# SavaRobotics/FoundationPose

Hardware: AMD Instinct MI355X
Metric: pose-hypotheses/sec (render+refine+score), 252 hyp x 160x160 (higher is better)
Workload: dtype f16

## Files before the change

foundationpose_amd/_lib.py:

```python
import ctypes
import os
import weakref
from ctypes import POINTER, Structure, byref, c_char_p, c_double, c_float, c_int, c_int64, c_uint, c_void_p

import numpy as np
import torch

_HERE = os.path.dirname(os.path.abspath(__file__))
LIB_PATH = os.path.join(_HERE, 'lib', 'libfoundationpose_amd.so')
_lib = None

FP_REFINE_SHARED_TRANSLATION = 1
FP_NET_REFINE, FP_NET_SCORE = 0, 1
FP_EINVAL = -1
FP_ERR_ADD, FP_ERR_ADDS, FP_ERR_ADD_SYM = 1, 2, 4
FP_BOP_MSSD, FP_BOP_MSPD = 1, 2
FP_VSD_MAX_TAUS = 32
FP_MESH_DIAMETER_MAX_POINTS = 1 << 21
FP_MESH_SIMPLIFY_MAX_VERTICES, FP_MESH_SIMPLIFY_MAX_FACES = 1 << 21, 1 << 23
FP_MESH_COMPONENTS_MAX_VERTICES, FP_MESH_COMPONENTS_MAX_FACES = 1 << 21, 1 << 23
FP_SCENE_MAX_INSTANCES = 1024
FP_SCENE_OCC_DEPTH, FP_SCENE_OCC_INSTANCES = 1, 2
FP_SCENE_INFO_COLS = 12
FP_SCENE_INFO_PX_COUNT_ALL, FP_SCENE_INFO_PX_COUNT_VALID, FP_SCENE_INFO_PX_COUNT_VISIB, FP_SCENE_INFO_PX_COUNT_IN_FRAME = 0, 1, 2, 3
# ... 138 lines not shown
  'fp_tsdf_integrate': (c_int, [c_void_p, c_void_p, c_void_p, c_void_p, c_void_p, c_int, c_int, c_int, c_void_p, c_void_p, c_float, c_void_p]),
  'fp_tsdf_extract_count': (c_int, [c_void_p, c_void_p, c_float, c_void_p, c_void_p]),
  'fp_tsdf_extract_write': (c_int, [c_void_p, c_void_p, c_void_p, c_void_p, c_void_p, c_void_p, c_int64, c_int64, c_void_p]),
  'fp_tsdf_read_plane': (c_int, [c_void_p, c_void_p, c_int, c_void_p, c_void_p]),
  'fp_tsdf_align': (c_int, [c_void_p, c_void_p, c_void_p, c_void_p, c_int, c_int, c_int, c_void_p, c_void_p, c_float, c_float, c_void_p, c_void_p, c_void_p]),
  'fp_texture_bake': (c_int, [c_void_p, c_void_p, c_int, c_void_p, c_int, c_void_p, c_void_p, c_void_p, c_void_p, c_int, c_int, c_int, c_void_p, c_void_p,
                              POINTER(FpTextureCfg), c_void_p, c_void_p, c_void_p, c_void_p]),
  'fp_point_mesh_distance': (c_int, [c_void_p, c_void_p, c_int, c_void_p, c_int, c_void_p, c_int, c_void_p, c_void_p, c_void_p, c_void_p]),
  'fp_distance_stats': (c_int, [c_void_p, c_void_p, c_int, c_void_p, c_int, c_void_p, c_void_p]),
  'fp_mesh_sample_surface': (c_int, [c_void_p, c_void_p, c_int, c_void_p, c_int, c_int, c_uint, c_void_p, c_void_p, c_void_p, c_void_p, c_void_p]),
  'fp_net_create': (c_int, [c_void_p, c_int, POINTER(FpTensor), c_int, c_int, POINTER(c_void_p)]),
  'fp_net_destroy': (c_int, [c_void_p]),
  'fp_net_rot_dim': (c_int, [c_void_p]),
  'fp_refine_forward': (c_int, [c_void_p, c_void_p, c_void_p, c_int, c_void_p, c_void_p, c_void_p]),
  'fp_net_tokens': (c_int, [c_void_p, c_void_p, c_void_p, c_int, c_void_p, c_void_p]),
  'fp_score_features': (c_int, [c_void_p, c_void_p, c_void_p, c_int, c_void_p, c_void_p]),
  'fp_score_tail': (c_int, [c_void_p, c_void_p, c_void_p, c_int, c_int, c_void_p, c_void_p, c_void_p]),
  'fp_score_tail_scores': (c_int, [c_void_p, c_void_p, c_void_p, c_int, c_int, c_int, c_float, c_void_p, c_void_p, c_void_p, c_void_p]),
  'fp_score_predict_rows_multi': (c_int, [c_void_p, c_void_p, POINTER(FpObjectBatch), c_int, c_double, c_int, c_void_p, c_void_p, c_void_p]),
  'fp_track_frame': (c_int, [c_void_p, POINTER(FpTrackArgs), c_void_p]),
  'fp_track_objects': (c_int, [c_void_p, POINTER(FpTrackObjectsArgs), c_void_p]),
  'fp_register_objects': (c_int, [c_void_p, POINTER(FpRegisterObjectsArgs), c_void_p]),
  'fp_mask_depth_stats_objects': (c_int, [c_void_p, c_void_p, c_void_p, c_void_p, c_void_p, c_int, c_int, c_int, c_float, c_void_p, c_void_p, c_void_p]),
  'fp_register_hypotheses': (c_int, [c_void_p, c_void_p, c_void_p, c_int, c_void_p, c_void_p, c_void_p, c_void_p, c_void_p]),
  'fp_register_rank': (c_int, [c_void_p, c_void_p, c_void_p, c_void_p, c_int, c_void_p, c_void_p, c_void_p, c_void_p, c_void_p, c_void_p]),
  'fp_pose_update': (c_int, [c_void_p, c_void_p, c_void_p, c_void_p, c_int, c_int, c_int, c_void_p, c_float, c_float, c_void_p, c_void_p]),
  'fp_pose_update_deepim': (c_int, [c_void_p, c_void_p, c_void_p, c_void_p, c_int, c_int, c_void_p, c_void_p, c_float, c_float, c_float, c_void_p, c_void_p]),
  'fp_refine_predict': (c_int, [c_void_p, c_void_p, c_void_p, c_void_p, c_void_p, c_int, c_int, c_void_p, c_double, POINTER(FpRefineCfg), c_void_p, c_int, c_int, c_void_p, c_void_p, c_void_p]),
  'fp_refine_predict_multi': (c_int, [c_void_p, c_void_p, POINTER(FpObjectBatch), c_int, POINTER(FpRefineCfg), c_void_p, c_int, c_void_p, c_void_p, c_void_p]),
  'fp_refine_predict_multi_flags': (c_int, [c_void_p, c_void_p, POINTER(FpObjectBatch), c_int, POINTER(FpRefineCfg), c_void_p, c_int, c_void_p, c_void_p, c_uint, c_void_p]),
  'fp_score_predict_features_multi': (c_int, [c_void_p, c_void_p, POINTER(FpObjectBatch), c_int, c_double, c_int, c_void_p, c_void_p, c_void_p]),
  'fp_score_predict_features': (c_int, [c_void_p, c_void_p, c_void_p, c_void_p, c_void_p, c_int, c_int, c_void_p, c_double, c_double, c_int, c_void_p, c_int, c_void_p, c_void_p]),
  'fp_conv3x3_band_f16': (c_int, [c_void_p, c_void_p, c_int, c_int, c_void_p, c_void_p, c_void_p, c_int, c_void_p, c_void_p]),
  'fp_conv2d_f16': (c_int, [c_void_p, c_void_p, c_int, c_int, c_int, c_int, c_void_p, c_void_p, c_int, c_int, c_int, c_int, c_int, c_void_p, c_int, c_void_p, c_int, c_void_p]),
  'fp_token_linear_f16': (c_int, [c_void_p, c_void_p, c_int, c_void_p, c_void_p, c_int, c_int, c_void_p, c_void_p, c_void_p, c_int, c_void_p, c_void_p]),
  'fp_head_mlp_f16': (c_int, [c_void_p, c_void_p, c_void_p, c_int] + [c_void_p] * 8 + [c_void_p, c_void_p]),
  'fp_attention_f16': (c_int, [c_void_p, c_void_p, c_void_p, c_int, c_int, c_void_p, c_void_p]),
  'fp_cluster_poses': (c_int, [c_float, c_float, c_void_p, c_int, c_void_p, c_int, c_void_p]),
  'fp_prof_enable': (c_int, [c_void_p, c_int]),
  'fp_prof_read': (c_int, [c_void_p, c_char_p, POINTER(c_double), POINTER(c_int64), POINTER(c_double)]),
  'fp_prof_read_busy': (c_int, [c_void_p, c_char_p, POINTER(c_double)]),
  'fp_prof_reset': (c_int, [c_void_p]),
}


def exported_symbols():
  return sorted(_PROTOS)


def lib():
  global _lib
  if _lib is None:
    if not os.path.exists(LIB_PATH):
      raise FoundationPoseAmdError(
        f'{LIB_PATH} is missing: build the HIP library first (python -c "import __graft_entry__ as g; g.build()" '
        f'or make -C foundationpose_amd/csrc).  foundationpose_amd has no CPU fallback.')
    L = ctypes.CDLL(LIB_PATH)
    for name, (res, args) in _PROTOS.items():
      fn = getattr(L, name)
      fn.restype = res
      fn.argtypes = args
    _lib = L
  return _lib


def check(rc):
# ... 180 lines not shown
```

foundationpose_amd/csrc/api.hip:

```cpp
#include "common.h"
#include <memory>
#include <cstring>

#include <cmath>
#include <cstdarg>
#include <cstdlib>
#include <algorithm>

static thread_local char g_err[1024] = "";

void fp_set_error(const char *fmt, ...) {
  va_list ap;
  va_start(ap, fmt);
  vsnprintf(g_err, sizeof(g_err), fmt, ap);
  va_end(ap);
}

extern "C" const char *fp_last_error(void) { return g_err; }
extern "C" int fp_version(void) { return 102; }

size_t fp_arena_bytes_for(int n_hyp) {
  return (size_t)n_hyp * (size_t)(17u << 20) + ((size_t)64 << 20);
}

size_t fp_arena_inner_bytes(int n_hyp) {
  return (size_t)n_hyp * (size_t)(15u << 20) + ((size_t)8 << 20) + (n_hyp <= 4 ? ((size_t)40 << 20) : 0);
}

int fp_arena_ensure(fp_ctx *ctx, size_t bytes) {
  Arena &a = ctx->arena;
  if (a.cap - a.off >= bytes && a.base) return FP_OK;
  if (a.off != 0) {
    fp_set_error("arena too small for a nested request of %zu bytes (cap %zu, used %zu); call fp_ctx_reserve first", bytes, a.cap, a.off);
    return FP_ENOMEM;
  }
  FP_CHECK_HIP(hipSetDevice(ctx->device));
  if (a.base) {
    FP_CHECK_HIP(hipDeviceSynchronize());
    FP_CHECK_HIP(hipFree(a.base));
    a.base = nullptr;
    a.cap = 0;
  }
  void *p = nullptr;
  hipError_t e = hipMalloc(&p, bytes);
  if (e != hipSuccess) {
    fp_set_error("hipMalloc(%zu) failed: %s", bytes, hipGetErrorString(e));
    return FP_ENOMEM;
  }
  a.base = (char *)p;
  a.cap = bytes;
  a.off = 0;
  ++a.generation;
  return FP_OK;
}

int fp_set_kernel_attributes(fp_ctx *ctx) {
  std::vector<KernelLds> v;
  conv_kernel_lds(v), conv_halo_kernel_lds(v), conv_s1b_kernel_lds(v), conv_small_kernel_lds(v), conv_s2_kernel_lds(v), stem_kernel_lds(v);
  tok_gemm_kernel_lds(v), tok_qkv_kernel_lds(v), head_mlp_kernel_lds(v), attn_kernel_lds(v), raster_kernel_lds(v);
  FP_CHECK_HIP(hipSetDevice(ctx->device));
  for (const KernelLds &k : v)
    if (k.bytes > 48 * 1024) FP_CHECK_HIP(hipFuncSetAttribute(k.fn, hipFuncAttributeMaxDynamicSharedMemorySize, k.bytes));
  return FP_OK;
}

extern "C" int fp_ctx_create(int device, fp_ctx **out) {
  FP_REQUIRE(out, "fp_ctx_create: null out");
  int n = 0;
  FP_CHECK_HIP(hipGetDeviceCount(&n));
  FP_REQUIRE(device >= 0 && device < n, "fp_ctx_create: device %d out of range (%d visible)", device, n);
  FP_CHECK_HIP(hipSetDevice(device));
  hipDeviceProp_t prop;
  FP_CHECK_HIP(hipGetDeviceProperties(&prop, device));
  fp_ctx *c = new fp_ctx;
  c->device = device;
  c->num_cu = prop.multiProcessorCount;
  if (hipMalloc(&c->zero_page, 4096 + FP_TAIL_MAX_GROUPS * sizeof(int)) != hipSuccess ||
      hipMemset(c->zero_page, 0, 4096 + FP_TAIL_MAX_GROUPS * sizeof(int)) != hipSuccess) {
    delete c;
    fp_set_error("fp_ctx_create: zero page allocation failed");
    return FP_ENOMEM;
  }
  c->tail_counter = (int *)((char *)c->zero_page + 4096);
  const int rc = fp_set_kernel_attributes(c);
  if (rc != FP_OK) {
    (void)hipFree(c->zero_page);
    delete c;
    return rc;
  }
  *out = c;
  return FP_OK;
// ... 1223 lines not shown
                             int Cout, int KH, int KW, int stride, int pad, const void *d_res, int relu, void *d_out, int out_f32,
                             void *stream) {
  FP_REQUIRE(ctx && d_in && d_w_packed && d_bias && d_out, "fp_conv2d_f16: null argument");
  FP_REQUIRE(stride >= 1 && pad >= 0 && Nimg >= 0, "fp_conv2d_f16: bad stride/pad/N");
  ConvArgs a = conv_args(d_in, d_w_packed, d_bias, d_res, d_out, Nimg, H, W, Cin, Cout, KH, KW, stride, pad, relu);
  a.out_mode = out_f32 ? 1 : 0;
  ArenaScope scope(ctx->arena);
  if (!out_f32 && conv_small_shape(a, ctx->num_cu)) {
    const size_t bytes = small_packed_halfs(Cout, Cin) * sizeof(f16);
    FP_TRY(fp_arena_ensure(ctx, bytes + 4096));
    f16 *pk = (f16 *)ctx->arena.take(bytes);
    if (!pk) return FP_ENOMEM;
    FP_TRY(small_pack_weights(a.w, Cout, Cin, a.Kpad, pk, (hipStream_t)stream));
    a.wsm = pk;
    return launch_conv(ctx, a, (hipStream_t)stream);
  }
  a.ksplit = out_f32 ? 0 : conv_ksplit(a, ctx->num_cu);
  if (a.ksplit > 1) {
    const size_t bytes = (size_t)a.ksplit * a.M * a.Cout * sizeof(float);
    FP_TRY(fp_arena_ensure(ctx, bytes + 4096));
    a.splitk = (float *)ctx->arena.take(bytes);
    return a.splitk ? launch_conv(ctx, a, (hipStream_t)stream) : FP_ENOMEM;
  }
  a.ksplit = 0;
  if (!out_f32 && a.M >= S2_MIN_PIXELS && s2_supported(a)) {
    const size_t bytes = s2_packed_halfs(Cout, Cin) * sizeof(f16);
    FP_TRY(fp_arena_ensure(ctx, bytes + 4096));
    f16 *pk = (f16 *)ctx->arena.take(bytes);
    if (!pk) return FP_ENOMEM;
    FP_TRY(s2_pack_weights(a.w, Cout, Cin, a.Kpad, pk, (hipStream_t)stream));
    a.wpk = pk;
    return launch_conv(ctx, a, (hipStream_t)stream);
  }
  return launch_conv(ctx, a, (hipStream_t)stream);
}

extern "C" int fp_conv3x3_band_f16(fp_ctx *ctx, const void *d_in, int Nimg, int C, const void *d_w_packed, const float *d_bias, const void *d_res,
                                   int relu, void *d_out, void *stream) {
  FP_REQUIRE(ctx && d_in && d_w_packed && d_bias && d_out && Nimg >= 0, "fp_conv3x3_band_f16: bad argument");
  FP_REQUIRE(C == 128 || C == 256, "fp_conv3x3_band_f16: C=%d (128 or 256)", C);
  ConvArgs a = conv_args(d_in, d_w_packed, d_bias, d_res, d_out, Nimg, 40, 40, C, C, 3, 3, 1, 1, relu);
  if (a.M == 0) return FP_OK;
  const size_t bytes = s2_packed_halfs(C, C) * sizeof(f16);
  FP_TRY(fp_arena_ensure(ctx, bytes + 4096));
  ArenaScope scope(ctx->arena);
  f16 *pk = (f16 *)ctx->arena.take(bytes);
  if (!pk) return FP_ENOMEM;
  FP_TRY(s2_pack_weights(a.w, C, C, a.Kpad, pk, (hipStream_t)stream, 2, 1));
  a.wpk = pk;
  return launch_conv_s1b(ctx, a, (hipStream_t)stream);
}

extern "C" int fp_attention_f16(fp_ctx *ctx, const void *d_qk, const void *d_vt, int B, int T, void *d_out, void *stream) {
  FP_REQUIRE(ctx && d_qk && d_vt && d_out, "fp_attention_f16: null argument");
  return launch_attention(ctx, (const f16 *)d_qk, (const f16 *)d_vt, B, T, (f16 *)d_out, (hipStream_t)stream);
}

extern "C" int fp_cluster_poses(float angle_diff_deg, float dist_diff_m, const float *in, int n_in, const float *sym, int n_sym,
                                float *out) {
  FP_REQUIRE(in && sym && out && n_in >= 1 && n_sym >= 1, "fp_cluster_poses: bad argument");
  const float radian_thres = angle_diff_deg / 180.0f * (float)M_PI;
  int n_out = 0;
  auto keep = [&](const float *p) {
    memcpy(out + (size_t)n_out * 16, p, 16 * sizeof(float));
    ++n_out;
  };
  keep(in);
// ... 28 lines not shown
```

foundationpose_amd/csrc/common.h:

```cpp
#pragma once
#include <hip/hip_runtime.h>
#include <stdint.h>
#include <stdio.h>
#include <stdlib.h>
#include <string.h>
#include <string>
#include <vector>
#include <map>

#include "../../include/foundationpose_amd.h"

typedef _Float16 f16;
typedef _Float16 half8 __attribute__((ext_vector_type(8)));
typedef _Float16 half4 __attribute__((ext_vector_type(4)));
typedef float floatx16 __attribute__((ext_vector_type(16)));
typedef float floatx4 __attribute__((ext_vector_type(4)));

void fp_set_error(const char *fmt, ...);

inline long long fp_env_int(const char *name, long long fallback) {
  const char *e = getenv(name);
  return e ? atoll(e) : fallback;
}
inline bool fp_env_set(const char *name) { return getenv(name) != nullptr; }
// ... 173 lines not shown
    if (!ctx->ev_pool.empty()) {
      e = ctx->ev_pool.back();
      ctx->ev_pool.pop_back();
    } else {
      (void)hipEventCreate(&e);
    }
    return e;
  }
  ~ProfScope() {
    if (on) {
      (void)hipEventRecord(ev.b, s);
      ctx->pending.push_back(ev);
    }
  }
};

#ifdef __HIPCC__
__device__ __forceinline__ int xcd_remap(int id, int nwg) {
  const int xcd = id & 7, slot = id >> 3;
  const int q = nwg >> 3, r = nwg & 7;
  return (xcd < r ? xcd * (q + 1) : r * (q + 1) + (xcd - r) * q) + slot;
}
#endif

struct KernelLds {
  const void *fn;
  int bytes;
};
void conv_kernel_lds(std::vector<KernelLds> &v);
void conv_halo_kernel_lds(std::vector<KernelLds> &v);
void conv_s1b_kernel_lds(std::vector<KernelLds> &v);
void conv_small_kernel_lds(std::vector<KernelLds> &v);
void conv_s2_kernel_lds(std::vector<KernelLds> &v);
void stem_kernel_lds(std::vector<KernelLds> &v);
void tok_gemm_kernel_lds(std::vector<KernelLds> &v);
void tok_qkv_kernel_lds(std::vector<KernelLds> &v);
void head_mlp_kernel_lds(std::vector<KernelLds> &v);
void attn_kernel_lds(std::vector<KernelLds> &v);
void raster_kernel_lds(std::vector<KernelLds> &v);
int fp_set_kernel_attributes(fp_ctx *ctx);

struct ConvArgs {
  const f16 *in;
  const f16 *w;
  const float *bias;
  const f16 *res;
  const float *post_add;
  void *out;
  int Nimg, H, W, Cin, Ho, Wo, Cout, KH, KW, stride, pad, Kpad, M;
  int relu, out_mode;
  int out_ld, split_m, coff_hi, post_period, tokens;
  float *splitk = nullptr;
  int ksplit = 0;
  const f16 *wpk = nullptr;
  const f16 *wsm = nullptr;
  int hyp = 0;
};
int launch_conv(fp_ctx *ctx, const ConvArgs &a, hipStream_t s);
#define S2_MIN_PIXELS 2000
bool s2_supported(const ConvArgs &a);
int s2_ct_for(int Cout);
size_t s2_packed_halfs(int Cout, int Cin);
int s2_pack_weights(const f16 *d_w, int Cout, int Cin, int Kpad, f16 *d_out, hipStream_t s, int ct_force = 0, int order = 0);
int launch_conv_s2(fp_ctx *ctx, const ConvArgs &a, hipStream_t s);
bool s1b_supported(const ConvArgs &a);
int launch_conv_s1b(fp_ctx *ctx, const ConvArgs &a, hipStream_t s);

bool conv_small_shape(const ConvArgs &a, int num_cu);
bool conv_small_use(const ConvArgs &a, int num_cu);
size_t small_packed_halfs(int Cout, int Cin);
int small_pack_weights(const f16 *d_w, int Cout, int Cin, int Kpad, f16 *d_out, hipStream_t s);
int launch_conv_small(fp_ctx *ctx, const ConvArgs &a, hipStream_t s);

__host__ __device__ __forceinline__ int vt_col(int t) { return (t & ~15) | (((t >> 2) & 1) << 3) | (((t >> 3) & 1) << 2) | (t & 3); }
int launch_attention(fp_ctx *ctx, const f16 *qk, const f16 *vt, int B, int T, f16 *out, hipStream_t s);

#define TG_MAXBLK 6
struct TokGemmBlock {
  const f16 *w;
  const float *bias;
  void *out;
  int ld, coff;
  int relu;
  int vt = 0;
};
struct TokGemmArgs {
  const f16 *in;
  int M, nblk, tokens;
  TokGemmBlock blk[TG_MAXBLK];
  const f16 *res;
  const float *gamma, *beta;
  float *gsum;
};
enum { TG_EPI_ROWS = 0, TG_EPI_VT = 1, TG_EPI_LN = 2, TG_EPI_LNSUM = 3 };
int launch_tok_gemm(fp_ctx *ctx, const TokGemmArgs &a, int epi, hipStream_t s);
int tok_qkv_small_max();
int launch_tok_qkv(fp_ctx *ctx, const TokGemmArgs &a, hipStream_t s, int hyp = 0);
// ... 166 lines not shown
```

foundationpose_amd/csrc/conv.hip:

```cpp
#include "common.h"
#include "device_util.h"
#include <cstdlib>
#include <type_traits>

#define CV_BK 32

#define C2_BN 256
#define C2_BK 32

#ifdef HALO_STAMP
__device__ unsigned long long g_igemm_stamps[4096 * 4 * 4];
extern "C" __attribute__((visibility("default"))) int fp_dbg_igemm_stamps(unsigned long long *host) {
  return hipMemcpyFromSymbol(host, HIP_SYMBOL(g_igemm_stamps), sizeof(g_igemm_stamps)) == hipSuccess ? 0 : -1;
}
#define ISTAMP(x) x
#else
#define ISTAMP(x)
#endif


template <int BM, int KW, bool CIN8, int NT, bool RES, bool SPLIT = false>
__device__ __forceinline__ void igemm2_tile(const ConvArgs &p, const f16 *__restrict__ zero_page, const int m0, const int c0, f16 *smem, const int ks = 0) {
  constexpr int TN = 64 * NT;
  constexpr int XH = TN * C2_BK, WH = BM * C2_BK;
// ... 410 lines not shown

bool conv_halo_supported(const ConvArgs &a);
int launch_conv_halo(fp_ctx *ctx, const ConvArgs &a, hipStream_t s);
bool stem_supported(const ConvArgs &a);
int launch_stem(fp_ctx *ctx, const ConvArgs &a, hipStream_t s);

int launch_conv(fp_ctx *ctx, const ConvArgs &a, hipStream_t s) {
  FP_REQUIRE(a.Cin == 8 || a.Cin % 32 == 0, "conv: Cin=%d must be 8 or a multiple of 32", a.Cin);
  FP_REQUIRE(a.Cout % 64 == 0, "conv: Cout=%d must be a multiple of 64", a.Cout);
  FP_REQUIRE(a.Kpad % CV_BK == 0 && a.Kpad >= a.KH * a.KW * a.Cin, "conv: bad Kpad=%d", a.Kpad);
  FP_REQUIRE(a.KH == a.KW && (a.KW == 1 || a.KW == 3 || a.KW == 7), "conv: kernel %dx%d unsupported (1,3,7)", a.KH, a.KW);
  FP_REQUIRE(a.M == a.Nimg * a.Ho * a.Wo, "conv: M mismatch");
  FP_REQUIRE(a.out_ld % 4 == 0 && a.coff_hi % 4 == 0, "conv: out_ld/coff must be multiples of 4");
  if (a.M == 0) return FP_OK;
  const double flops = 2.0 * (double)a.M * a.Cout * a.KH * a.KW * (a.Cin == 8 ? 6 : a.Cin);
  const bool halo = conv_halo_supported(a);
  const char *cls = halo ? "conv3x3_halo" : (a.KW == 3) ? "conv3x3_s2" : (a.KW == 7 ? "conv7x7" : "linear");
  ProfScope ps(ctx, s, cls, flops);
  if (!(a.splitk && a.ksplit > 1) && conv_small_use(a, ctx->num_cu)) return launch_conv_small(ctx, a, s);
  {
    static const int band = fp_env_int("FP_C128_BAND", 1);
    if (band != 0 && (a.Cin == 128 || band == 2) && (long long)a.M > (long long)ctx->num_cu * 512 && s1b_supported(a)) return launch_conv_s1b(ctx, a, s);
  }
  if (halo) return launch_conv_halo(ctx, a, s);
  if (a.splitk && a.ksplit > 1) {
    FP_REQUIRE(a.KW == 3 && a.stride == 2 && a.Cout % 128 == 0 && (a.Kpad / C2_BK) % a.ksplit == 0 && a.out_mode == 0, "conv split-K: unsupported layer");
    const int n_t = ((a.M + 63) / 64) * (a.Cout / 128);
    hipLaunchKernelGGL((conv_igemm2_splitk_kernel<128, 3>), dim3(n_t * a.ksplit), dim3(256), igemm2_lds_bytes<128>(), s, a, (const f16 *)ctx->zero_page);
    FP_CHECK_HIP(hipGetLastError());
    return launch_splitk_finish(a, s);
  }
  if (stem_supported(a)) return launch_stem(ctx, a, s);
  if (a.wpk && a.M >= S2_MIN_PIXELS && s2_supported(a)) return launch_conv_s2(ctx, a, s);
  const bool bm128 = (a.Cout % 128 == 0);
  const f16 *zp = (const f16 *)ctx->zero_page;
  if (a.Cin == 8) {
    FP_REQUIRE(a.KW == 7, "conv: Cin=8 path is the 7x7 stem");
    return bm128 ? launch_two<128, 7, true>(ctx, a, zp, s) : launch_two<64, 7, true>(ctx, a, zp, s);
  }
  if (a.KW == 3) return bm128 ? launch_two<128, 3, false>(ctx, a, zp, s) : launch_two<64, 3, false>(ctx, a, zp, s);
  if (a.KW == 1) return bm128 ? launch_two<128, 1, false>(ctx, a, zp, s) : launch_two<64, 1, false>(ctx, a, zp, s);
  FP_REQUIRE(false, "conv: unsupported configuration KW=%d Cin=%d", a.KW, a.Cin);
}
```

foundationpose_amd/csrc/conv_s2.hip:

```cpp
#include "common.h"
#include "device_util.h"

#define S2_THREADS 256
#define S2_STAGE_PAD 8

template <int WO, int ROWS, int CT>
struct S2Cfg {
  static constexpr int P = 42;
  static_assert(WO == 20, "pitch chosen for 20-wide outputs");
  static constexpr int BROWS = 2 * ROWS + 2;
  static constexpr int NPT = ROWS * WO / 32;
  static constexpr int BAND_INSTR = ((BROWS * P + 31) / 32 + 3) / 4 * 4;
  static constexpr int BAND_BYTES = BAND_INSTR * 1024;
  static constexpr int DPW = BAND_INSTR / 4;
  static constexpr int STAGE_LD = CT * 32 + S2_STAGE_PAD;
  static constexpr int LDS_BYTES = 2 * BAND_BYTES;
  static_assert(ROWS * WO == NPT * 32 && (2 * P - WO) % 16 == 0 && P >= 2 * WO + 1, "tile / pitch");
  static_assert(4 * 32 * STAGE_LD * 2 <= BAND_BYTES, "epilogue staging fits one band buffer");
};

__global__ void s2_pack_kernel(const f16 *__restrict__ w, int Cin, int Kpad, int CT, size_t total, f16 *__restrict__ out, int order) {
  const size_t idx = (size_t)blockIdx.x * blockDim.x + threadIdx.x;
  if (idx >= total) return;
  const int e = idx & 7, lane = (idx >> 3) & 63;
  size_t rest = idx >> 9;
  const int nch = Cin / 16;
  const int ct = rest % CT;
  rest /= CT;
  int tap, chunk;
  if (order == 1) {
    const int ks = rest % 2;
    rest /= 2;
    tap = rest % 9;
    rest /= 9;
    chunk = (int)(rest % (nch / 2)) * 2 + ks;
    rest /= nch / 2;
  } else {
    tap = rest % 9;
    rest /= 9;
    chunk = rest % nch;
    rest /= nch;
  }
  const int co = ((int)rest * CT + ct) * 32 + (lane & 31);
  const int k = tap * Cin + chunk * 16 + (lane >> 5) * 8 + e;
  out[idx] = w[(size_t)co * Kpad + k];
}

template <int WO, int ROWS, int CT>
__global__ __launch_bounds__(S2_THREADS, 2) void conv3x3_s2_kernel(ConvArgs p, const f16 *__restrict__ wpk, const f16 *__restrict__ zero_page,
                                                                    int n_tiles, int n_cob) {
  using C = S2Cfg<WO, ROWS, CT>;
  constexpr int HO = WO, HI = 2 * WO, WI = 2 * WO, P = C::P, NPT = C::NPT, DPW = C::DPW;
  extern __shared__ __attribute__((aligned(16))) unsigned char s2_smem[];
  const int tid = threadIdx.x, lane = tid & 63, wave = __builtin_amdgcn_readfirstlane(tid >> 6);
  const int lr = lane & 31, lh = lane >> 5;
  const unsigned lds0 = (unsigned)(size_t)(__attribute__((address_space(3))) void *)s2_smem;

  const int tile = xcd_remap(blockIdx.x, n_tiles);
  const int cb = tile % n_cob, pt = tile / n_cob;
  const int g0 = pt * ROWS;
  const int img0 = g0 / HO, oy0 = g0 - img0 * HO;
  const int jb = HO - oy0;
  const int nch = p.Cin >> 4;

  unsigned src_off[DPW];
#pragma unroll
  for (int v = 0; v < DPW; ++v) {
    const int q = (wave + 4 * v) * 32 + (lane >> 1), hl = (lane & 1) ^ ((q >> 3) & 1);
    const int b = q / P, c = q - b * P;
// ... 156 lines not shown
```

foundationpose_amd/csrc/net.hip:

```cpp
#include "common.h"
#include "device_util.h"

#include <algorithm>
#include <cmath>
#include <cstdlib>
#include <memory>

struct ConvW {
  f16 *w = nullptr;
  f16 *wpk = nullptr;
  f16 *wsm = nullptr;
  float *bias = nullptr;
  int Cin = 0, Cout = 0, K = 1, Kpad = 0, stride = 1;
};

struct LinP {
  f16 *w = nullptr;
  float *bias = nullptr;
};

struct HeadW {
  LinP q, k, v, out, ff1, ff2;
  float *ln1g = nullptr, *ln1b = nullptr, *ln2g = nullptr, *ln2b = nullptr, *hw = nullptr, *hb = nullptr;
  int out_dim = 0;
};

struct LinF32 {
  float *w = nullptr, *b = nullptr, *wt = nullptr;
  int N = 0, K = 0;
};

struct fp_net {
  int kind = 0, use_bn = 1;
  ConvW trunk[15];
  float *pe = nullptr;
  HeadW heads[2];
  LinP att_q, att_k, att_v;
  LinF32 att_out;
  float *tail_wqk_t = nullptr, *tail_bqk = nullptr;
  double *tail_u = nullptr, *tail_c = nullptr, tail_b_eff = 0.0;
  std::vector<void *> allocs;
};

// ... 65 lines not shown
    FP_TRY(need(sd, bnkey + ".bias", 1, {Cout}, &be));
    FP_TRY(need(sd, bnkey + ".running_mean", 1, {Cout}, &mu));
    FP_TRY(need(sd, bnkey + ".running_var", 1, {Cout}, &var));
    for (int c = 0; c < Cout; ++c) {
      scale[c] = g->data[c] / std::sqrt(var->data[c] + 1e-5f);
      shift[c] = be->data[c] - mu->data[c] * scale[c];
    }
  }
  const int CinP = (Cin < 8) ? 8 : Cin;
  FP_REQUIRE(CinP == 8 || CinP % 32 == 0, "conv '%s': Cin=%d unsupported", wkey.c_str(), Cin);
  const int Kraw = K * K * CinP, Kpad = (Kraw + 31) / 32 * 32;
  std::vector<f16> hw((size_t)Cout * Kpad, (f16)0.f);
  std::vector<float> hb(Cout);
  for (int co = 0; co < Cout; ++co) {
    for (int ci = 0; ci < Cin; ++ci)
      for (int ky = 0; ky < K; ++ky)
        for (int kx = 0; kx < K; ++kx)
          hw[(size_t)co * Kpad + (ky * K + kx) * CinP + ci] = (f16)(w->data[(((size_t)co * Cin + ci) * K + ky) * K + kx] * scale[co]);
    hb[co] = b->data[co] * scale[co] + shift[co];
  }
  out->Cin = CinP;
  out->Cout = Cout;
  out->K = K;
  out->Kpad = Kpad;
  out->stride = stride;
  FP_TRY(upload(net, hw, &out->w));
  FP_TRY(upload(net, hb, &out->bias));
  if (K == 3 && (stride == 2 || (stride == 1 && CinP == Cout && (Cout == 128 || Cout == 256))) && CinP % 16 == 0 && s2_ct_for(Cout) != 0) {
    void *pk = nullptr;
    FP_CHECK_HIP(hipMalloc(&pk, s2_packed_halfs(Cout, CinP) * sizeof(f16)));
    net->allocs.push_back(pk);
    out->wpk = (f16 *)pk;
    FP_TRY(s2_pack_weights(out->w, Cout, CinP, Kpad, out->wpk, nullptr, stride == 1 ? 2 : 0, stride == 1 ? 1 : 0));
    FP_CHECK_HIP(hipStreamSynchronize(nullptr));
  }
  if (K == 3 && ((stride == 1 && (CinP == 128 || CinP == 256 || CinP == 512)) || (stride == 2 && (CinP == 256 || CinP == 64))) && Cout % 32 == 0 && Kpad == 9 * CinP) {
    void *pk = nullptr;
    FP_CHECK_HIP(hipMalloc(&pk, small_packed_halfs(Cout, CinP) * sizeof(f16)));
    net->allocs.push_back(pk);
    out->wsm = (f16 *)pk;
    FP_TRY(small_pack_weights(out->w, Cout, CinP, Kpad, out->wsm, nullptr));
    FP_CHECK_HIP(hipStreamSynchronize(nullptr));
  }
  return FP_OK;
}

void pack_tok_weights(const float *w, f16 *out) {
  for (int wave = 0; wave < 4; ++wave)
    for (int k16 = 0; k16 < 32; ++k16)
      for (int i = 0; i < 4; ++i)
        for (int lane = 0; lane < 64; ++lane) {
          const int lr = lane & 31, lh = lane >> 5;
          const float *src = w + (size_t)(wave * 128 + i * 32 + lr) * 512 + k16 * 16 + lh * 8;
          f16 *dst = out + ((((size_t)wave * 32 + k16) * 4 + i) * 64 + lane) * 8;
          for (int e = 0; e < 8; ++e) dst[e] = (f16)src[e];
        }
}

int make_linear(fp_net *net, const SD &sd, const std::string &wkey, const std::string &bkey, int r0, LinP *out) {
  const fp_tensor *w, *b;
  FP_TRY(need(sd, wkey, 2, {-1, 512}, &w));
  FP_TRY(need(sd, bkey, 1, {w->shape[0]}, &b));
  FP_REQUIRE(r0 + 512 <= w->shape[0], "linear '%s': rows out of range", wkey.c_str());
  std::vector<f16> hw((size_t)512 * 512);
  std::vector<float> hb(512);
  pack_tok_weights(w->data + (size_t)r0 * 512, hw.data());
// ... 144 lines not shown
  if (!net) return FP_OK;
  for (void *p : net->allocs) (void)hipFree(p);
  delete net;
  return FP_OK;
}

extern "C" int fp_net_rot_dim(const fp_net *net) { return (net && net->kind == FP_NET_REFINE) ? net->heads[1].out_dim : 0; }

int conv_ksplit(const ConvArgs &a, int num_cu);

namespace {

struct Conv2dCall {
  const f16 *in;
  int Nimg, H, W;
  const ConvW *cw;
  const f16 *res = nullptr;
  int relu = 1;
  void *out = nullptr;
  int out_mode = 0;
  int out_ld = 0, split_m = 0x7fffffff, coff_hi = 0;
  const float *post_add = nullptr;
  int post_period = 1;
  int tokens = 400;
};

int run_conv(fp_ctx *ctx, const Conv2dCall &c, hipStream_t s, float *splitk_scratch = nullptr, int hyp = 0) {
  ConvArgs a;
  const ConvW &w = *c.cw;
  a.in = c.in;
  a.w = w.w;
  a.wpk = w.wpk;
  a.wsm = w.wsm;
  a.hyp = hyp;
  a.bias = w.bias;
  a.res = c.res;
  a.post_add = c.post_add;
  a.out = c.out;
  a.Nimg = c.Nimg;
  a.H = c.H;
  a.W = c.W;
  a.Cin = w.Cin;
  a.KH = a.KW = w.K;
  a.stride = w.stride;
  a.pad = (w.K - 1) / 2;
  a.Ho = (c.H + 2 * a.pad - w.K) / w.stride + 1;
  a.Wo = (c.W + 2 * a.pad - w.K) / w.stride + 1;
  a.Cout = w.Cout;
  a.Kpad = w.Kpad;
  a.M = c.Nimg * a.Ho * a.Wo;
  a.relu = c.relu;
  a.out_mode = c.out_mode;
  a.out_ld = c.out_ld ? c.out_ld : w.Cout;
  a.split_m = c.split_m;
  a.coff_hi = c.coff_hi;
  a.post_period = c.post_period;
  a.tokens = c.tokens;
  if (splitk_scratch) {
    a.ksplit = conv_ksplit(a, ctx->num_cu);
    a.splitk = a.ksplit > 1 ? splitk_scratch : nullptr;
  }
  return launch_conv(ctx, a, s);
}

#define TAKE(ptr, type, count)                                                            \
  type *ptr = (type *)ctx->arena.take((size_t)(count) * sizeof(type));                    \
// ... 406 lines not shown
```

include/foundationpose_amd.h:

```cpp
#ifndef FOUNDATIONPOSE_AMD_H
#define FOUNDATIONPOSE_AMD_H

#include <stddef.h>
#include <stdint.h>

#ifdef __cplusplus
extern "C" {
#endif

#pragma GCC visibility push(default)

#define FP_OK 0
#define FP_EINVAL (-1)
#define FP_EHIP (-2)
#define FP_ENOMEM (-3)
#define FP_EKEY (-4)

typedef struct fp_ctx fp_ctx;
typedef struct fp_mesh fp_mesh;
typedef struct fp_net fp_net;

const char *fp_last_error(void);
int fp_version(void);

// ... 318 lines not shown
  int tex_size, top_n;
  float depth_tol , cos_min, zfar;
} fp_texture_cfg;
int fp_texture_bake(fp_ctx *ctx, const float *d_pos, int V, const int32_t *d_faces, int F, const uint8_t *d_vertex_colors,
                    const uint8_t *d_rgb, const float *d_depth, const uint8_t *d_mask, int n_views, int H, int W, const double *K,
                    const double *cam_in_ob, const fp_texture_cfg *cfg, uint8_t *d_texture, float *d_uv, int8_t *d_used, void *stream);

#define FP_SURFDIST_MAX_POINTS (1 << 24)
#define FP_SURFDIST_MAX_FACES (1 << 23)
#define FP_SURFDIST_MAX_TAUS 8
#define FP_SURFDIST_MAX_SAMPLES (1 << 22)
#define FP_SURFDIST_TILE 1024
#define FP_SURFDIST_CHUNK 256
int fp_point_mesh_distance(fp_ctx *ctx, const float *d_points, int n, const float *d_pos, int V, const int32_t *d_faces, int F,
                           float *d_dist, int32_t *d_face, float *d_closest, void *stream);

#define FP_SURFDIST_STATS_COUNT 0
#define FP_SURFDIST_STATS_SUM 1
#define FP_SURFDIST_STATS_SUM_SQ 2
#define FP_SURFDIST_STATS_MAX 3
#define FP_SURFDIST_STATS_NOT_FINITE 4
#define FP_SURFDIST_STATS_TAU0 5
int fp_distance_stats(fp_ctx *ctx, const float *d_dist, int n, const double *h_taus, int n_taus, double *d_stats, void *stream);

int fp_mesh_sample_surface(fp_ctx *ctx, const float *d_pos, int V, const int32_t *d_faces, int F, int n, uint32_t seed, float *d_points,
                           int32_t *d_face, float *d_bary, int64_t *d_area_q, void *stream);

int fp_conv2d_f16(fp_ctx *ctx, const void *d_in, int Nimg, int H, int W, int Cin, const void *d_w_packed, const float *d_bias,
                  int Cout, int KH, int KW, int stride, int pad, const void *d_res, int relu, void *d_out, int out_f32,
                  void *stream);

int fp_conv3x3_band_f16(fp_ctx *ctx, const void *d_in, int Nimg, int C, const void *d_w_packed, const float *d_bias, const void *d_res,
                        int relu, void *d_out, void *stream);
int fp_attention_f16(fp_ctx *ctx, const void *d_qk, const void *d_vt, int B, int T, void *d_out, void *stream);

int fp_token_linear_f16(fp_ctx *ctx, const void *d_in, int M, const float *h_weight, const float *h_bias, int epilogue, int relu,
                        const void *d_res, const float *h_gamma, const float *h_beta, int tokens, void *d_out, void *stream);

int fp_head_mlp_f16(fp_ctx *ctx, const void *d_att, const void *d_tok, int M, const float *h_w_out, const float *h_b_out,
                    const float *h_gamma1, const float *h_beta1, const float *h_w1, const float *h_b1, const float *h_w2,
                    const float *h_b2, float *d_gsum, void *stream);

int fp_cluster_poses(float angle_diff_deg, float dist_diff_m, const float *h_poses_in, int n_in, const float *h_symmetry_tfs,
                     int n_sym, float *h_out);

int fp_prof_enable(fp_ctx *ctx, int on);
int fp_prof_read(fp_ctx *ctx, const char *kernel_class, double *total_ms, int64_t *launches, double *flops);
int fp_prof_read_busy(fp_ctx *ctx, const char *kernel_class, double *busy_ms);
int fp_prof_reset(fp_ctx *ctx);

#pragma GCC visibility pop

#ifdef __cplusplus
}
#endif
#endif
```

Baseline: 7382.

## Add row-band MFMA kernel for 3x3 stride-2 64→128 conv at 80x80

Adds a specialized kernel for the 3x3 stride-2 conv (64→128 channels, 80x80→40x40). It loads a swizzled input band into LDS once per tile and streams pre-packed weights from registers with a lookahead queue, running 32x32x16 MFMAs. The epilogue stages results through LDS so global stores are coalesced. At net load it packs weights in a new order and routes the layer to this kernel when there are enough images. The trade-off is another specialized code path, extra packed weight memory, and an env toggle.

```diff
diff --git a/foundationpose_amd/_lib.py b/foundationpose_amd/_lib.py
--- a/foundationpose_amd/_lib.py
+++ b/foundationpose_amd/_lib.py
@@ -194,6 +194,7 @@
   'fp_score_predict_features_multi': (c_int, [c_void_p, c_void_p, POINTER(FpObjectBatch), c_int, c_double, c_int, c_void_p, c_void_p, c_void_p]),
   'fp_score_predict_features': (c_int, [c_void_p, c_void_p, c_void_p, c_void_p, c_void_p, c_int, c_int, c_void_p, c_double, c_double, c_int, c_void_p, c_int, c_void_p, c_void_p]),
   'fp_conv3x3_band_f16': (c_int, [c_void_p, c_void_p, c_int, c_int, c_void_p, c_void_p, c_void_p, c_int, c_void_p, c_void_p]),
+  'fp_conv3x3_s2_rows_f16': (c_int, [c_void_p, c_void_p, c_int, c_void_p, c_void_p, c_int, c_void_p, c_void_p]),
   'fp_conv2d_f16': (c_int, [c_void_p, c_void_p, c_int, c_int, c_int, c_int, c_void_p, c_void_p, c_int, c_int, c_int, c_int, c_int, c_void_p, c_int, c_void_p, c_int, c_void_p]),
   'fp_token_linear_f16': (c_int, [c_void_p, c_void_p, c_int, c_void_p, c_void_p, c_int, c_int, c_void_p, c_void_p, c_void_p, c_int, c_void_p, c_void_p]),
   'fp_head_mlp_f16': (c_int, [c_void_p, c_void_p, c_void_p, c_int] + [c_void_p] * 8 + [c_void_p, c_void_p]),
diff --git a/foundationpose_amd/csrc/api.hip b/foundationpose_amd/csrc/api.hip
--- a/foundationpose_amd/csrc/api.hip
+++ b/foundationpose_amd/csrc/api.hip
@@ -56,7 +56,7 @@
 
 int fp_set_kernel_attributes(fp_ctx *ctx) {
   std::vector<KernelLds> v;
-  conv_kernel_lds(v), conv_halo_kernel_lds(v), conv_s1b_kernel_lds(v), conv_small_kernel_lds(v), conv_s2_kernel_lds(v), stem_kernel_lds(v);
+  conv_kernel_lds(v), conv_halo_kernel_lds(v), conv_s1b_kernel_lds(v), conv_small_kernel_lds(v), conv_s2_kernel_lds(v), conv_s2r_kernel_lds(v), stem_kernel_lds(v);
   tok_gemm_kernel_lds(v), tok_qkv_kernel_lds(v), head_mlp_kernel_lds(v), attn_kernel_lds(v), raster_kernel_lds(v);
   FP_CHECK_HIP(hipSetDevice(ctx->device));
   for (const KernelLds &k : v)
@@ -1346,7 +1346,32 @@
     a.wpk = pk;
     return launch_conv(ctx, a, (hipStream_t)stream);
   }
+  if (!out_f32 && Nimg >= S2R_MIN_IMAGES && s2r_supported(a)) {
+    const size_t bytes = s2r_packed_halfs() * sizeof(f16);
+    FP_TRY(fp_arena_ensure(ctx, bytes + 4096));
+    f16 *pk = (f16 *)ctx->arena.take(bytes);
+    if (!pk) return FP_ENOMEM;
+    FP_TRY(s2r_pack_weights(a.w, pk, (hipStream_t)stream));
+    a.wrw = pk;
+    return launch_conv(ctx, a, (hipStream_t)stream);
+  }
   return launch_conv(ctx, a, (hipStream_t)stream);
+}
+
+extern "C" int fp_conv3x3_s2_rows_f16(fp_ctx *ctx, const void *d_in, int Nimg, const void *d_w_packed, const float *d_bias, int relu, void *d_out,
+                                      void *stream) {
+  FP_REQUIRE(ctx && d_in && d_w_packed && d_bias && d_out && Nimg >= 0, "fp_conv3x3_s2_rows_f16: bad argument");
+  FP_REQUIRE((long long)Nimg * 1600 <= 0x7fffffffLL / 128, "fp_conv3x3_s2_rows_f16: Nimg=%d too large", Nimg);
+  ConvArgs a = conv_args(d_in, d_w_packed, d_bias, nullptr, d_out, Nimg, 80, 80, 64, 128, 3, 3, 2, 1, relu);
+  if (a.M == 0) return FP_OK;
+  const size_t bytes = s2r_packed_halfs() * sizeof(f16);
+  FP_TRY(fp_arena_ensure(ctx, bytes + 4096));
+  ArenaScope scope(ctx->arena);
+  f16 *pk = (f16 *)ctx->arena.take(bytes);
+  if (!pk) return FP_ENOMEM;
+  FP_TRY(s2r_pack_weights(a.w, pk, (hipStream_t)stream));
+  a.wrw = pk;
+  return launch_conv_s2r(ctx, a, (hipStream_t)stream);
 }
 
 extern "C" int fp_conv3x3_band_f16(fp_ctx *ctx, const void *d_in, int Nimg, int C, const void *d_w_packed, const float *d_bias, const void *d_res,
diff --git a/foundationpose_amd/csrc/common.h b/foundationpose_amd/csrc/common.h
--- a/foundationpose_amd/csrc/common.h
+++ b/foundationpose_amd/csrc/common.h
@@ -229,6 +229,7 @@
 void conv_s1b_kernel_lds(std::vector<KernelLds> &v);
 void conv_small_kernel_lds(std::vector<KernelLds> &v);
 void conv_s2_kernel_lds(std::vector<KernelLds> &v);
+void conv_s2r_kernel_lds(std::vector<KernelLds> &v);
 void stem_kernel_lds(std::vector<KernelLds> &v);
 void tok_gemm_kernel_lds(std::vector<KernelLds> &v);
 void tok_qkv_kernel_lds(std::vector<KernelLds> &v);
@@ -251,6 +252,7 @@
   int ksplit = 0;
   const f16 *wpk = nullptr;
   const f16 *wsm = nullptr;
+  const f16 *wrw = nullptr;
   int hyp = 0;
 };
 int launch_conv(fp_ctx *ctx, const ConvArgs &a, hipStream_t s);
@@ -260,6 +262,12 @@
 size_t s2_packed_halfs(int Cout, int Cin);
 int s2_pack_weights(const f16 *d_w, int Cout, int Cin, int Kpad, f16 *d_out, hipStream_t s, int ct_force = 0, int order = 0);
 int launch_conv_s2(fp_ctx *ctx, const ConvArgs &a, hipStream_t s);
+#define S2R_MIN_IMAGES 3
+bool s2r_supported(const ConvArgs &a);
+bool s2r_use(const ConvArgs &a);
+size_t s2r_packed_halfs();
+int s2r_pack_weights(const f16 *d_w, f16 *d_out, hipStream_t s);
+int launch_conv_s2r(fp_ctx *ctx, const ConvArgs &a, hipStream_t s);
 bool s1b_supported(const ConvArgs &a);
 int launch_conv_s1b(fp_ctx *ctx, const ConvArgs &a, hipStream_t s);
 
diff --git a/foundationpose_amd/csrc/conv.hip b/foundationpose_amd/csrc/conv.hip
--- a/foundationpose_amd/csrc/conv.hip
+++ b/foundationpose_amd/csrc/conv.hip
@@ -466,6 +466,7 @@
   }
   if (stem_supported(a)) return launch_stem(ctx, a, s);
   if (a.wpk && a.M >= S2_MIN_PIXELS && s2_supported(a)) return launch_conv_s2(ctx, a, s);
+  if (s2r_use(a)) return launch_conv_s2r(ctx, a, s);
   const bool bm128 = (a.Cout % 128 == 0);
   const f16 *zp = (const f16 *)ctx->zero_page;
   if (a.Cin == 8) {
diff --git a/foundationpose_amd/csrc/conv_s2.hip b/foundationpose_amd/csrc/conv_s2.hip
--- a/foundationpose_amd/csrc/conv_s2.hip
+++ b/foundationpose_amd/csrc/conv_s2.hip
@@ -35,6 +35,11 @@
     rest /= 9;
     chunk = (int)(rest % (nch / 2)) * 2 + ks;
     rest /= nch / 2;
+  } else if (order == 2) {
+    chunk = rest % nch;
+    rest /= nch;
+    tap = rest % 9;
+    rest /= 9;
   } else {
     tap = rest % 9;
     rest /= 9;
diff --git a/foundationpose_amd/csrc/conv_s2r.hip b/foundationpose_amd/csrc/conv_s2r.hip
--- /dev/null
+++ b/foundationpose_amd/csrc/conv_s2r.hip
@@ -0,0 +1,154 @@
+#include "common.h"
+#include "device_util.h"
+
+#define S2R_THREADS 256
+
+namespace {
+
+constexpr int R_HO = 40, R_HI = 80;
+constexpr int R_TR = 16, R_TC = 8;
+constexpr int R_CG = R_HO / R_TC;
+constexpr int R_P = 2 * R_TC + 1;
+constexpr int R_BROWS = 2 * R_TR + 2;
+constexpr int R_INSTR = ((R_BROWS * R_P + 7) / 8 + 3) / 4 * 4;
+constexpr int R_DPW = R_INSTR / 4;
+constexpr int R_BAND_BYTES = R_INSTR * 1024;
+constexpr int R_STAGE_LD = 128 + 8;
+constexpr int R_STEPS = 9 * 4;
+constexpr int R_AHEAD = 6;
+static_assert(R_TR * R_TC * R_STAGE_LD * 2 <= R_BAND_BYTES, "epilogue staging fits the band");
+static_assert(2 * R_BAND_BYTES <= 160 * 1024, "two workgroups per CU");
+static_assert(R_HO % R_TC == 0 && R_TR < R_HO, "a tile touches at most two images");
+
+__device__ __forceinline__ int r_swz(int b, int c) { return ((b >> 1) & 3) | (((c >> 1) & 1) << 2); }
+
+}
+
+__global__ __launch_bounds__(S2R_THREADS, 2) void conv3x3_s2_rows_kernel(ConvArgs p, const f16 *__restrict__ wpk, const f16 *__restrict__ zero_page,
+                                                                         int n_tiles) {
+  extern __shared__ __attribute__((aligned(16))) unsigned char s2r_smem[];
+  const int tid = threadIdx.x, lane = tid & 63, wave = __builtin_amdgcn_readfirstlane(tid >> 6);
+  const int lr = lane & 31, lh = lane >> 5;
+  const int wm = wave >> 1, wn = wave & 1;
+  const unsigned lds0 = (unsigned)(size_t)(__attribute__((address_space(3))) void *)s2r_smem;
+
+  const int tile = xcd_remap(blockIdx.x, n_tiles);
+  const int cg = tile % R_CG, rgp = tile / R_CG;
+  const int g0 = rgp * R_TR;
+  const int img0 = g0 / R_HO, oy0 = g0 - img0 * R_HO, ox0 = cg * R_TC;
+  const int jb = R_HO - oy0;
+
+#pragma unroll
+  for (int v = 0; v < R_DPW; ++v) {
+    const int u = wave + 4 * v, q = u * 8 + (lane >> 3);
+    const int b = q / R_P, c = q - b * R_P;
+    const int ch = (lane & 7) ^ r_swz(b, c);
+    const int ix = c < R_TC ? 2 * (ox0 + c) : 2 * (ox0 + c - R_TC) - 1;
+    const bool second = b > 2 * jb;
+    const int img = img0 + (second ? 1 : 0), iy = second ? b - 2 * jb - 2 : 2 * oy0 + b - 1;
+    const bool ok = b < R_BROWS && iy >= 0 && iy < R_HI && ix >= 0 && ix < R_HI && img < p.Nimg;
+    const char *src = ok ? (const char *)p.in + ((size_t)((img * R_HI + iy) * R_HI + ix) * 64 + ch * 8) * 2 : (const char *)zero_page;
+    glds16(src, lds0 + u * 1024);
+  }
+
+  const half8 *wp = reinterpret_cast<const half8 *>(wpk) + (size_t)wm * (R_STEPS * 2 * 64) + lane;
+  half8 aq[R_AHEAD][2];
+#pragma unroll
+  for (int d = 0; d < R_AHEAD; ++d)
+#pragma unroll
+    for (int ct = 0; ct < 2; ++ct) aq[d][ct] = wp[(d * 2 + ct) * 64];
+
+  floatx16 acc[2][2];
+  acc_from_bias<2, 2>(acc, p.bias, wm * 64, lh);
+
+  const int ox = lr & 7;
+  int rb[2];
+#pragma unroll
+  for (int j = 0; j < 2; ++j) {
+    const int jr = ((2 * wn + j) * 32 + lr) >> 3;
+    rb[j] = 2 * jr + (jr >= jb ? 1 : 0);
+  }
+  auto b_read = [&](int i, int j) __attribute__((always_inline)) -> half8 {
+    const int t = i >> 2, s = i & 3, ky = t / 3, kx = t - ky * 3;
+    const int b = rb[j] + ky, c = ox + (kx == 1 ? 0 : R_TC + (kx == 2 ? 1 : 0));
+    return *reinterpret_cast<const half8 *>(s2r_smem + ((b * R_P + c) << 7) + (((2 * s + lh) ^ r_swz(b, c)) << 4));
+  };
+
+  wait_vm_lgkm<0>();
+  __builtin_amdgcn_s_barrier();
+  __builtin_amdgcn_sched_barrier(0);
+
+  half8 bq[2][2];
+#pragma unroll
+  for (int j = 0; j < 2; ++j) bq[0][j] = b_read(0, j);
+#pragma unroll
+  for (int i = 0; i < R_STEPS; ++i) {
+    if (i + 1 < R_STEPS) {
+#pragma unroll
+      for (int j = 0; j < 2; ++j) bq[(i + 1) & 1][j] = b_read(i + 1, j);
+    }
+    __builtin_amdgcn_sched_barrier(0);
+#pragma unroll
+    for (int j = 0; j < 2; ++j)
+#pragma unroll
+      for (int ct = 0; ct < 2; ++ct) acc[ct][j] = __builtin_amdgcn_mfma_f32_32x32x16_f16(aq[i % R_AHEAD][ct], bq[i & 1][j], acc[ct][j], 0, 0, 0);
+    __builtin_amdgcn_sched_barrier(0);
+    if (i + R_AHEAD < R_STEPS) {
+#pragma unroll
+      for (int ct = 0; ct < 2; ++ct) aq[i % R_AHEAD][ct] = wp[((i + R_AHEAD) * 2 + ct) * 64];
+    }
+    __builtin_amdgcn_sched_barrier(0);
+  }
+  __syncthreads();
+
+  f16 *stage = reinterpret_cast<f16 *>(s2r_smem);
+#pragma unroll
+  for (int j = 0; j < 2; ++j) {
+    const int pl = (2 * wn + j) * 32 + lr;
+#pragma unroll
+    for (int ct = 0; ct < 2; ++ct)
+#pragma unroll
+      for (int rg = 0; rg < 4; ++rg) {
+        half4 hv;
+#pragma unroll
+        for (int e = 0; e < 4; ++e) hv[e] = (f16)acc[ct][j][rg * 4 + e];
+        if (p.relu) hv = __builtin_elementwise_max(hv, half4{(f16)0.f, (f16)0.f, (f16)0.f, (f16)0.f});
+        *reinterpret_cast<half4 *>(&stage[pl * R_STAGE_LD + wm * 64 + ct * 32 + rg * 8 + lh * 4]) = hv;
+      }
+  }
+  __syncthreads();
+  const int rows = p.Nimg * R_HO;
+  uint4 ov[8];
+#pragma unroll
+  for (int u = 0; u < 8; ++u) ov[u] = *reinterpret_cast<const uint4 *>(&stage[(u * 16 + (tid >> 4)) * R_STAGE_LD + (tid & 15) * 8]);
+#pragma unroll
+  for (int u = 0; u < 8; ++u) {
+    const int pl = u * 16 + (tid >> 4), g = g0 + (pl >> 3);
+    if (g < rows) *reinterpret_cast<uint4 *>((f16 *)p.out + ((size_t)g * R_HO + ox0 + (pl & 7)) * 128 + (tid & 15) * 8) = ov[u];
+  }
+}
+
+bool s2r_supported(const ConvArgs &a) {
+  return a.KH == 3 && a.KW == 3 && a.stride == 2 && a.pad == 1 && a.out_mode == 0 && !a.res && !a.post_add && a.out_ld == a.Cout && a.split_m >= a.M &&
+         a.H == R_HI && a.W == R_HI && a.Ho == R_HO && a.Wo == R_HO && a.Cin == 64 && a.Cout == 128 && a.Kpad == 9 * 64 && !(a.splitk && a.ksplit > 1);
+}
+
+bool s2r_use(const ConvArgs &a) {
+  static const int on = fp_env_int("FP_S2_ROWS", 1);
+  return on != 0 && a.wrw != nullptr && a.Nimg >= S2R_MIN_IMAGES && (a.hyp == 0 || a.hyp >= S2R_MIN_IMAGES) && s2r_supported(a);
+}
+
+size_t s2r_packed_halfs() { return s2_packed_halfs(128, 64); }
+
+int s2r_pack_weights(const f16 *d_w, f16 *d_out, hipStream_t s) { return s2_pack_weights(d_w, 128, 64, 9 * 64, d_out, s, 2, 2); }
+
+void conv_s2r_kernel_lds(std::vector<KernelLds> &v) { v.push_back({(const void *)conv3x3_s2_rows_kernel, R_BAND_BYTES}); }
+
+int launch_conv_s2r(fp_ctx *ctx, const ConvArgs &a, hipStream_t s) {
+  FP_REQUIRE(a.wrw && s2r_supported(a), "launch_conv_s2r: unsupported layer or no packed weights");
+  if (a.M == 0) return FP_OK;
+  const int n_tiles = (a.Nimg * R_HO + R_TR - 1) / R_TR * R_CG;
+  hipLaunchKernelGGL(conv3x3_s2_rows_kernel, dim3(n_tiles), dim3(S2R_THREADS), R_BAND_BYTES, s, a, a.wrw, (const f16 *)ctx->zero_page, n_tiles);
+  FP_CHECK_HIP(hipGetLastError());
+  return FP_OK;
+}
diff --git a/foundationpose_amd/csrc/net.hip b/foundationpose_amd/csrc/net.hip
--- a/foundationpose_amd/csrc/net.hip
+++ b/foundationpose_amd/csrc/net.hip
@@ -9,6 +9,7 @@
 struct ConvW {
   f16 *w = nullptr;
   f16 *wpk = nullptr;
+  f16 *wrw = nullptr;
   f16 *wsm = nullptr;
   float *bias = nullptr;
   int Cin = 0, Cout = 0, K = 1, Kpad = 0, stride = 1;
@@ -140,6 +141,14 @@
     net->allocs.push_back(pk);
     out->wpk = (f16 *)pk;
     FP_TRY(s2_pack_weights(out->w, Cout, CinP, Kpad, out->wpk, nullptr, stride == 1 ? 2 : 0, stride == 1 ? 1 : 0));
+    FP_CHECK_HIP(hipStreamSynchronize(nullptr));
+  }
+  if (K == 3 && stride == 2 && CinP == 64 && Cout == 128 && Kpad == 9 * 64) {
+    void *pk = nullptr;
+    FP_CHECK_HIP(hipMalloc(&pk, s2r_packed_halfs() * sizeof(f16)));
+    net->allocs.push_back(pk);
+    out->wrw = (f16 *)pk;
+    FP_TRY(s2r_pack_weights(out->w, out->wrw, nullptr));
     FP_CHECK_HIP(hipStreamSynchronize(nullptr));
   }
   if (K == 3 && ((stride == 1 && (CinP == 128 || CinP == 256 || CinP == 512)) || (stride == 2 && (CinP == 256 || CinP == 64))) && Cout % 32 == 0 && Kpad == 9 * CinP) {
@@ -350,6 +359,7 @@
   a.w = w.w;
   a.wpk = w.wpk;
   a.wsm = w.wsm;
+  a.wrw = w.wrw;
   a.hyp = hyp;
   a.bias = w.bias;
   a.res = c.res;
diff --git a/include/foundationpose_amd.h b/include/foundationpose_amd.h
--- a/include/foundationpose_amd.h
+++ b/include/foundationpose_amd.h
@@ -374,6 +374,8 @@
 
 int fp_conv3x3_band_f16(fp_ctx *ctx, const void *d_in, int Nimg, int C, const void *d_w_packed, const float *d_bias, const void *d_res,
                         int relu, void *d_out, void *stream);
+int fp_conv3x3_s2_rows_f16(fp_ctx *ctx, const void *d_in, int Nimg, const void *d_w_packed, const float *d_bias, int relu, void *d_out,
+                           void *stream);
 int fp_attention_f16(fp_ctx *ctx, const void *d_qk, const void *d_vt, int B, int T, void *d_out, void *stream);
 
 int fp_token_linear_f16(fp_ctx *ctx, const void *d_in, int M, const float *h_weight, const float *h_bias, int epilogue, int relu,
```

New measurement: 7411 (median of 6 runs). No clear change (+0.4%).
